# rafaelvp-db/databricks-distributed-deep-learning

Hardware: AMD Instinct MI355X
Metric: ResNet-50 images/sec (whole node) (higher is better)
Workload: dtype bf16

## Files before the change

### csrc/build.py

```python
#!/usr/bin/env python3
from __future__ import annotations

import argparse
import concurrent.futures as cf
import glob
import os
import shutil
import subprocess
import sys

ROOT = os.path.dirname(os.path.dirname(os.path.abspath(__file__)))
CSRC = os.path.join(ROOT, "csrc")
BUILD = os.path.join(ROOT, "build", "native")
OUT_DIR = os.path.join(ROOT, "databricks_distributed_deep_learning_amd", "_native")
OUT = os.path.join(OUT_DIR, "libddl_kernels.so")
HIPCC = os.environ.get("HIPCC", "/opt/rocm/bin/hipcc")
ARCH = os.environ.get("DDL_OFFLOAD_ARCH", "gfx950")

COMMON = ["-O3", "-std=c++17", "-fPIC", f"--offload-arch={ARCH}", "-I", os.path.join(CSRC, "include"),
          "-Wno-unused-result", "-ffp-contract=fast", "-munsafe-fp-atomics"]


def sources():
    return sorted(glob.glob(os.path.join(CSRC, "kernels", "*.hip"))) + \
        sorted(glob.glob(os.path.join(CSRC, "runtime", "*.cpp")))


def headers():
    return glob.glob(os.path.join(CSRC, "include", "*.h")) + glob.glob(os.path.join(CSRC, "kernels", "*.h"))


def obj_for(src):
    return os.path.join(BUILD, os.path.basename(src) + ".o")


def needs(src, obj, hdr_mtime):
    if not os.path.exists(obj):
        return True
    m = os.path.getmtime(obj)
    return os.path.getmtime(src) > m or hdr_mtime > m


_VGPR_FORM = ["-mllvm", "-amdgpu-mfma-vgpr-form"]
EXTRA = {"gemm_big.hip": _VGPR_FORM, "conv3x3.hip": _VGPR_FORM, "skinny_gemm.hip": _VGPR_FORM,
         "stream_gemm.hip": _VGPR_FORM, "gemm_duo.hip": _VGPR_FORM, "conv3_bwd.hip": _VGPR_FORM}


GEMM_SOURCES = ["gemm.hip", "gemm_big.hip", "gemm_duo.hip", "skinny_gemm.hip", "stream_gemm.hip", "conv3x3.hip",
                "conv3_bwd.hip"]


def gemm_src_hash() -> str:
    import hashlib
    h = hashlib.sha256()
    for path in [os.path.join(CSRC, "kernels", n) for n in GEMM_SOURCES] + \
            sorted(glob.glob(os.path.join(CSRC, "include", "*.h"))):
        h.update(os.path.basename(path).encode())
        with open(path, "rb") as f:
            h.update(f.read())
    return h.hexdigest()[:16]


def buildinfo_obj() -> str:
    digest = gemm_src_hash()
    src = os.path.join(BUILD, "buildinfo.cpp")
    obj = src + ".o"
    text = ('extern "C" __attribute__((visibility("default"))) const char* ddl_gemm_src_hash() '
            f'{{ return "{digest}"; }}\n')
    old = open(src).read() if os.path.exists(src) else ""
    if old != text or not os.path.exists(obj):
        with open(src, "w") as f:
            f.write(text)
        r = subprocess.run(["g++", "-O2", "-fPIC", "-c", src, "-o", obj], capture_output=True, text=True)
        if r.returncode != 0:
            raise RuntimeError(f"buildinfo compile failed: {r.stderr}")
    return obj


# ... 63 lines not shown
```

### databricks_distributed_deep_learning_amd/models/layers.py

```python
from __future__ import annotations

import math
from typing import Optional

import torch
import torch.nn as nn

from .. import ops
from ..ops.bridge import BNStats


class Conv2d(nn.Module):

    def __init__(self, cin: int, cout: int, k: int, stride: int = 1, padding: int = 0):
        super().__init__()
        self.cin, self.cout, self.k, self.stride, self.padding = cin, cout, k, stride, padding
        self.weight = nn.Parameter(torch.empty(cout, k, k, cin))
        std = math.sqrt(2.0 / (cout * k * k))
        nn.init.normal_(self.weight, 0.0, std)

    def forward(self, x, grad_residual=None, bn_stats=None, grad_to=None):
        return ops.conv2d(x, self.weight, self.stride, self.padding, grad_residual=grad_residual, bn_stats=bn_stats,
                          grad_to=grad_to)

    def extra_repr(self):
        return f"{self.cin}, {self.cout}, k={self.k}, stride={self.stride}, padding={self.padding}"


class BatchNorm2d(nn.Module):

    def __init__(self, c: int, eps: float = 1e-5, momentum: float = 0.1, relu: bool = False,
                 zero_init: bool = False):
        super().__init__()
        self.c, self.eps, self.momentum, self.relu = c, eps, momentum, relu
        self.weight = nn.Parameter(torch.zeros(c) if zero_init else torch.ones(c))
        self.bias = nn.Parameter(torch.zeros(c))
        self.register_buffer("running_mean", torch.zeros(c))
        self.register_buffer("running_var", torch.ones(c))
        self.register_buffer("num_batches_tracked", torch.tensor(0, dtype=torch.long))
        self._nbt_pending = 0
        self.sync_group = None

    def _flush_nbt(self):
        if self._nbt_pending:
            self.num_batches_tracked.add_(self._nbt_pending)
            self._nbt_pending = 0

    def _save_to_state_dict(self, destination, prefix, keep_vars):
        self._flush_nbt()
        super()._save_to_state_dict(destination, prefix, keep_vars)

    def _load_from_state_dict(self, state_dict, prefix, *args, **kwargs):
        self._nbt_pending = 0
        super()._load_from_state_dict(state_dict, prefix, *args, **kwargs)

    def forward(self, x, residual: Optional[torch.Tensor] = None, residual_grad_to=None, stats=None):
        if self.training:
            self._nbt_pending += 1
        return ops.batch_norm(x, self.weight, self.bias, self.running_mean, self.running_var,
                              self.training, self.momentum, self.eps, self.relu, residual,
                              residual_grad_to=residual_grad_to, stats=stats, group=self.sync_group)

    def _apply(self, fn, recurse=True):
        rm, rv = self.running_mean, self.running_var
        super()._apply(fn, recurse)
        if self.running_mean.dtype != torch.float32:
            self.running_mean = self.running_mean.float()
            self.running_var = self.running_var.float()
        return self

    def extra_repr(self):
        return f"{self.c}, eps={self.eps}, relu={self.relu}"


class Linear(nn.Module):
    def __init__(self, fin: int, fout: int, bias: bool = True, act: Optional[str] = None,
                 init_std: Optional[float] = None):
        super().__init__()
        self.fin, self.fout, self.act = fin, fout, act
        self.weight = nn.Parameter(torch.empty(fout, fin))
        self.bias = nn.Parameter(torch.zeros(fout)) if bias else None
        if init_std is not None:
            nn.init.normal_(self.weight, 0.0, init_std)
        else:
            nn.init.kaiming_uniform_(self.weight, a=math.sqrt(5))
            if self.bias is not None:
                bound = 1.0 / math.sqrt(fin)
                nn.init.uniform_(self.bias, -bound, bound)

    def forward(self, x, grad_residual=None, fuse_dgelu: bool = False, residual=None, residual_grad_to=None):
        return ops.linear(x, self.weight, self.bias, self.act, grad_residual=grad_residual, fuse_dgelu=fuse_dgelu,
                          residual=residual, residual_grad_to=residual_grad_to)

    def extra_repr(self):
        return f"{self.fin}, {self.fout}, bias={self.bias is not None}, act={self.act}"


def conv_bn(conv: "Conv2d", bn: "BatchNorm2d", x, residual=None, grad_residual=None, residual_grad_to=None,
            grad_to=None):
    st = BNStats() if bn.training else None
    y = conv(x, grad_residual=grad_residual, bn_stats=st, grad_to=grad_to)
    return bn(y, residual=residual, residual_grad_to=residual_grad_to, stats=st)


def conv_stats(conv: "Conv2d", bn: "BatchNorm2d", x, grad_residual=None):
    st = BNStats() if bn.training else None
    return conv(x, grad_residual=grad_residual, bn_stats=st), st


def conv_bn_add_bn(conv: "Conv2d", bn: "BatchNorm2d", x, bn2: "BatchNorm2d", y2, st2=None):
    st = BNStats() if bn.training else None
    y = conv(x, bn_stats=st)
    if bn.training and bn2.training and bn.sync_group is None and bn2.sync_group is None and bn.relu \
            and not bn2.relu:
        out = ops.batch_norm_add_bn(y, bn.weight, bn.bias, bn.running_mean, bn.running_var, bn.momentum, bn.eps,
                                    y2, bn2.weight, bn2.bias, bn2.running_mean, bn2.running_var, bn2.momentum,
                                    bn2.eps, st, st2)
        if out is not None:
            bn._nbt_pending += 1
            bn2._nbt_pending += 1
            return out
    return bn(y, residual=bn2(y2, stats=st2), stats=st)


def conv_bn_maxpool(conv: "Conv2d", bn: "BatchNorm2d", x):
    if bn.training and bn.sync_group is None and bn.relu:
        st = BNStats()
        y = conv(x, bn_stats=st)
        out = ops.bn_relu_maxpool(y, bn.weight, bn.bias, bn.running_mean, bn.running_var, bn.momentum, bn.eps, st)
        if out is not None:
            bn._nbt_pending += 1
            return out
        return ops.max_pool2d(bn(y, stats=st), 3, 2, 1)
    return ops.max_pool2d(conv_bn(conv, bn, x), 3, 2, 1)

# ... 49 lines not shown
```

### databricks_distributed_deep_learning_amd/models/resnet.py

```python
from __future__ import annotations

import os
from typing import List, Optional, Type, Union

import torch
import torch.nn as nn

from .. import ops
from ..ops.bridge import GradBridge
from .layers import BatchNorm2d, Conv2d, Linear, conv_bn, conv_bn_add_bn, conv_bn_maxpool, conv_stats


_BRIDGE = os.environ.get("DDL_GRAD_BRIDGE", "1") != "0"


def _bridge(x: torch.Tensor, training: bool):
    return GradBridge() if (_BRIDGE and training and torch.is_grad_enabled() and x.requires_grad) else None


class BasicBlock(nn.Module):
    expansion = 1

    def __init__(self, cin: int, planes: int, stride: int = 1, downsample: Optional[nn.Module] = None,
                 zero_init_residual: bool = False):
        super().__init__()
        self.conv1 = Conv2d(cin, planes, 3, stride, 1)
        self.bn1 = BatchNorm2d(planes, relu=True)
        self.conv2 = Conv2d(planes, planes, 3, 1, 1)
        self.bn2 = BatchNorm2d(planes, relu=True, zero_init=zero_init_residual)
        self.downsample = downsample

    def forward(self, x):
        if self.downsample is None:
            br = _bridge(x, self.training)
            out = conv_bn(self.conv1, self.bn1, x, grad_residual=br)
            return conv_bn(self.conv2, self.bn2, out, residual=x, residual_grad_to=br)
        br = _bridge(x, self.training)
        y_id, st_id = self.downsample.conv_stats(x, grad_residual=br)
        out = conv_bn(self.conv1, self.bn1, x, grad_to=br)
        return conv_bn_add_bn(self.conv2, self.bn2, out, self.downsample.bn, y_id, st_id)


class Bottleneck(nn.Module):
    expansion = 4

    def __init__(self, cin: int, planes: int, stride: int = 1, downsample: Optional[nn.Module] = None,
                 zero_init_residual: bool = False):
        super().__init__()
        self.conv1 = Conv2d(cin, planes, 1)
        self.bn1 = BatchNorm2d(planes, relu=True)
        self.conv2 = Conv2d(planes, planes, 3, stride, 1)
        self.bn2 = BatchNorm2d(planes, relu=True)
        self.conv3 = Conv2d(planes, planes * 4, 1)
        self.bn3 = BatchNorm2d(planes * 4, relu=True, zero_init=zero_init_residual)
        self.downsample = downsample

    def forward(self, x):
        if self.downsample is None:
            br = _bridge(x, self.training)
            out = conv_bn(self.conv1, self.bn1, x, grad_residual=br)
            out = conv_bn(self.conv2, self.bn2, out)
            return conv_bn(self.conv3, self.bn3, out, residual=x, residual_grad_to=br)
        br = _bridge(x, self.training)
        y_id, st_id = self.downsample.conv_stats(x, grad_residual=br)
        out = conv_bn(self.conv1, self.bn1, x, grad_to=br)
        out = conv_bn(self.conv2, self.bn2, out)
        return conv_bn_add_bn(self.conv3, self.bn3, out, self.downsample.bn, y_id, st_id)


class Downsample(nn.Module):

    def __init__(self, cin: int, cout: int, stride: int):
        super().__init__()
        self.add_module("0", Conv2d(cin, cout, 1, stride, 0))
        self.add_module("1", BatchNorm2d(cout, relu=False))

    @property
    def bn(self):
        return self._modules["1"]

    def conv_stats(self, x, grad_residual=None):
        return conv_stats(self._modules["0"], self._modules["1"], x, grad_residual=grad_residual)

    def forward(self, x, grad_residual=None):
        return conv_bn(self._modules["0"], self._modules["1"], x, grad_residual=grad_residual)


class ResNet(nn.Module):
    def __init__(self, block: Type[Union[BasicBlock, Bottleneck]], layers: List[int], num_classes: int = 1000,
                 zero_init_residual: bool = False, channels_last_input: bool = True):
        super().__init__()
        self.channels_last_input = channels_last_input
        self.inplanes = 64
        self.conv1 = Conv2d(3, 64, 7, 2, 3)
        self.bn1 = BatchNorm2d(64, relu=True)
        self.layer1 = self._make_layer(block, 64, layers[0], 1, zero_init_residual)
        self.layer2 = self._make_layer(block, 128, layers[1], 2, zero_init_residual)
        self.layer3 = self._make_layer(block, 256, layers[2], 2, zero_init_residual)
        self.layer4 = self._make_layer(block, 512, layers[3], 2, zero_init_residual)
        self.fc = Linear(512 * block.expansion, num_classes)

    def _make_layer(self, block, planes, blocks, stride, zir):
        down = None
        if stride != 1 or self.inplanes != planes * block.expansion:
            down = Downsample(self.inplanes, planes * block.expansion, stride)
        mods = [block(self.inplanes, planes, stride, down, zir)]
        self.inplanes = planes * block.expansion
        for _ in range(1, blocks):
            mods.append(block(self.inplanes, planes, 1, None, zir))
        return nn.Sequential(*mods)

    _ddl_direct_reads = ("conv1", "bn1")

    def features(self, x):
        if not self.channels_last_input:
            x = x.permute(0, 2, 3, 1).contiguous()
        x = conv_bn_maxpool(self.conv1, self.bn1, x)
        x = self.layer4(self.layer3(self.layer2(self.layer1(x))))
        return ops.global_avg_pool(x)

    def forward(self, x):
        return self.fc(self.features(x))


def resnet18(num_classes: int = 1000, **kw) -> ResNet:
    return ResNet(BasicBlock, [2, 2, 2, 2], num_classes, **kw)


def resnet34(num_classes: int = 1000, **kw) -> ResNet:
    return ResNet(BasicBlock, [3, 4, 6, 3], num_classes, **kw)


def resnet50(num_classes: int = 1000, **kw) -> ResNet:
    return ResNet(Bottleneck, [3, 4, 6, 3], num_classes, **kw)


def resnet101(num_classes: int = 1000, **kw) -> ResNet:
    return ResNet(Bottleneck, [3, 4, 23, 3], num_classes, **kw)


def resnet152(num_classes: int = 1000, **kw) -> ResNet:
    return ResNet(Bottleneck, [3, 8, 36, 3], num_classes, **kw)
# ... 19 lines not shown
```

### databricks_distributed_deep_learning_amd/ops/_lib.py

```python
from __future__ import annotations

import ctypes
import os
from typing import Optional

import torch

_PKG_DIR = os.path.dirname(os.path.dirname(os.path.abspath(__file__)))
LIB_PATH = os.environ.get("DDL_NATIVE_LIB") or os.path.join(_PKG_DIR, "_native", "libddl_kernels.so")

_lib: Optional[ctypes.CDLL] = None
_load_error: Optional[str] = None
_mode = os.environ.get("DDL_NATIVE", "auto").lower()


class NativeUnavailable(RuntimeError):
    pass


def set_mode(mode: str) -> None:
    global _mode
    if mode not in ("auto", "on", "off"):
        raise ValueError(mode)
    _mode = mode
# ... 90 lines not shown
    "ddl_bn_relu_maxpool": [I, P, P, P, P, P, P, I, I, I, I, I, I, P],
    "ddl_bn_bwd_pool_nblk": [],
    "ddl_bn_bwd_pool": [I, P, P, P, P, P, P, P, I, I, I, I, I, I, P, P, P, P, P, I, P],
    "ddl_bn_bwd_coef_from_partials": [I, P, I, P, L, P, P, L, I, P, P, P, I, P],
    "ddl_bn_bwd_apply_coef": [I, P, P, P, P, P, L, I, P, P],
    "ddl_bn_fwd_from_partials": [I, P, I, L, I, P, P, P, P, F, F, P, P, P, P, P, L],
    "ddl_conv_w_dgrad": [P, P, I, I, I, I, I, I, P, P, P],
    "ddl_conv_w_dgrad_batch": [P, P, I, P],
    "ddl_gelu_bwd_colsum": [I, P, P, P, L, I, P, P, I, I, P],
    "ddl_acc_f32": [I, P, P, L, P],
    "ddl_tanh_bwd": [I, P, P, P, L, P],
    "ddl_copy2d": [I, P, L, L, L, P, L, L, L, P],
    "ddl_add_into": [I, P, P, L, P],
    "ddl_zero": [P, L, P],
    "ddl_rows_add_row": [I, P, P, P, L, L, P],
    "ddl_seq_prepend_add": [I, P, P, P, P, L, L, L, P],
    "ddl_sort_ids_ok": [L, L],
    "ddl_sort_ids": [P, L, P, P, P],
    "ddl_drain_acc": [I, P, P, L, P],
    "ddl_acc_grad": [I, P, P, L, I, I, P],
    "ddl_softmax_topk": [I, P, L, I, I, P, P, P, P],
    "ddl_gemm_conv_multi": [I, I, P, P, P, P, P, L, I, P, P],
    "ddl_conv3x3": [P, P, P, I, I, I, I, I, P, P, P, P, P, P, I, P],
    "ddl_conv3x3_wgrad": [P, P, P, I, I, I, I, I, P, L, I, I, I, P],
    "ddl_stem_wgrad": [P, P, P, I, I, I, I, I, I, I, P, L, I, I, I, P],
    "ddl_stem_fwd": [P, P, P, I, I, I, I, P, I, P],
    "ddl_s2d_input": [P, I, I, I, I, I, P, I, I, P],
    "ddl_s2d_weight": [P, I, I, I, I, P, I, I, P],
    "ddl_skinny_gemm": [P, P, P, L, I, I, P, P, P, P, P, P, I, P],
    "ddl_stream_gemm": [P, P, P, L, I, I, P, P, P, P, P, P, I, P],
    "ddl_stream_wgrad_ws": [I, I],
    "ddl_conv3_bwd_grid": [L, I],
    "ddl_conv3_bwd": [P, P, P, P, P, P, P, P, P, P, P, P, P, P, L, P, I, I, L, I, I, I, P],
    "ddl_bn_bwd": [I, P, P, P, P, P, P, L, I, I, P, P, P, P, P, P, I, P],
    "ddl_ln_supported": [I],
    "ddl_ln_fwd": [I, P, P, L, P, P, P, P, P, L, I, F, U64, F, P],
    "ddl_ln_bwd_nblk": [L],
    "ddl_ln_bwd": [I, P, P, P, L, P, P, P, P, P, P, P, L, I, I, P, U64, F, P, P, P, P],
    "ddl_gelu_fwd": [I, P, P, L, P],
    "ddl_gelu_bwd": [I, P, P, P, L, P],
    "ddl_dropout": [I, P, P, L, U64, F, P],
    "ddl_colsum_nblk": [L],
    "ddl_colsum": [I, P, L, I, P, P, I, I, P],
    "ddl_softmax_ce": [I, P, P, L, I, P, P, P, P],
    "ddl_scale_by": [I, P, P, P, L, P],
    "ddl_maxpool_fwd": [I, P, P, P, I, I, I, I, I, I, I, I, I, P],
    "ddl_maxpool_bwd": [I, P, P, P, I, I, I, I, I, I, I, I, I, P],
    "ddl_avgpool_fwd": [I, P, P, I, I, I, P],
    "ddl_avgpool_bwd": [I, P, P, I, I, I, P],
    "ddl_embedding_fwd": [I, P, P, P, L, I, P],
    "ddl_embedding_bwd": [I, P, P, P, P, L, L, I, I, P],
    "ddl_embedding_bwd_sorted": [I, P, P, P, P, P, L, I, I, P],
    "ddl_sgd_step": [I, P, P, I, P, P, P, I, P, F, F, F, I, I, P],
    "ddl_adamw_step": [I, P, P, I, P, P, P, P, I, P, F, F, F, F, F, F, F, F, F, P],
    "ddl_lamb_step": [I, P, P, I, P, P, P, P, I, P, F, F, F, F, F, F, F, F, F, P, P],
    "ddl_sumsq": [I, P, L, P, P],
    "ddl_lamb_phase1": [I, P, P, P, P, P, I, P, F, F, F, F, F, F, F, F, P, P],
    "ddl_lamb_phase2": [P, I, P, P, P, P, I, F, F, F, F, F, P, P],
}
_fns = {}


def fn(name: str):
    f = _fns.get(name)
    if f is None:
        f = getattr(get(), name)
# ... 85 lines not shown
```

### databricks_distributed_deep_learning_amd/ops/_native_conv.py

```python
from __future__ import annotations

import ctypes
import os

import torch
import torch.nn.functional as F

from . import _lib
from ._lib import grad_ready, grad_sink
from ._native_gemm import MODE_CONV, MODE_CONVW, MODE_NN, MODE_NT, MODE_TN, gemm, plan, stats_rows_max
from ._native_norm import _BN_BWD_EPI, _BN_BWD_EPI_RES


def _desc(N, H, W, C, P, Q, stride, h_off, w_off, h_step, w_step, R, S, OH, OW, ostep=1, oa=0, ob=0):
    return [N, H, W, C, P, Q, stride, h_off, w_off, h_step, w_step, R, S, OH, OW, ostep, oa, ob]


STATS_MIN_K = int(os.environ.get("DDL_BN_STATS_MIN_K", "0"))
_DGRAD_NT = os.environ.get("DDL_DGRAD_NT", "1") != "0"


_CONV3X3 = os.environ.get("DDL_CONV3X3", "1") != "0"


# ... 406 lines not shown
    if sink is not None and (not sink.is_contiguous() or sink.dtype not in (torch.bfloat16, torch.float32)):
        return None
    wt = _w_dgrad(w, [0], [0], param).view(C, K)
    dx = torch.empty(N, H, W_, C, dtype=x.dtype, device=x.device)
    dw = sink if sink is not None else torch.empty(K, 1, 1, C, dtype=x.dtype, device=x.device)
    G = _lib.fn("ddl_conv3_bwd_grid")(M, 0)
    part = torch.empty(max(stats_rows_max(M), 1024) * 2 * C + 64 * C, dtype=torch.float32, device=x.device)
    wpart = torch.empty(G * K * C, dtype=torch.bfloat16, device=x.device)
    rc = _lib.fn("ddl_conv3_bwd")(dz.data_ptr(), x3.data_ptr(), mean3.data_ptr(), istd3.data_ptr(), coef.data_ptr(),
                                  x.data_ptr(), bnb.x.data_ptr(), _lib.p(bnb.mask), bnb.mean.data_ptr(),
                                  bnb.istd.data_ptr(), wt.data_ptr(), dx.data_ptr(), part.data_ptr(),
                                  wpart.data_ptr(), wpart.numel(), dw.data_ptr(), int(dw.dtype == torch.float32),
                                  int(sink is not None), M, K, C, 0, _lib.stream())
    if rc == -1:
        return None
    if rc < 0:
        raise RuntimeError(f"ddl_conv3_bwd failed: {rc}")
    bnb.set(dx, part, rc)
    return dx, (None if sink is not None else dw)


def _conv3_materialise(parked, dy):
    from .bridge import Conv3Fold
    dz, x3, mean3, istd3, coef = parked
    C = x3.shape[-1]
    dx3 = torch.empty_like(x3)
    _lib.call("ddl_bn_bwd_apply_coef", 1, dz.data_ptr(), x3.data_ptr(), mean3.data_ptr(), istd3.data_ptr(),
              coef.data_ptr(), x3.numel() // C, C, dx3.data_ptr())
    if Conv3Fold.is_parked(parked, dy):
        return dx3
    return (dy - dz.view_as(dy)) + dx3.view_as(dy)


class _Conv(torch.autograd.Function):
    @staticmethod
    def forward(ctx, x, w, stride, pad, bridge=None, stats=None, grad_to=None):
        ctx.w_param = w
        ctx.bridge = bridge
        ctx.grad_to = grad_to
        ctx.c3 = None
        ctx.bnb = getattr(x, "_ddl_bnb", None) if grad_to is None else None
        x = x.contiguous()
        w = w.contiguous()
        ctx.stride, ctx.pad = stride, pad
        ctx.save_for_backward(x, w)
        y = _fwd(x, w, stride, pad, stats=stats)
        if _conv3_fold_ok(x, w, stride, pad) and y.is_contiguous():
            from .bridge import Conv3Fold
            ctx.c3 = y._ddl_c3 = Conv3Fold()
        return y

    @staticmethod
    def backward(ctx, dy):
        x, w = ctx.saved_tensors
        dy = dy.contiguous()
        dx = dw = None
        parked = ctx.c3.take() if ctx.c3 is not None else None
        if parked is not None:
            from .bridge import Conv3Fold
            if (Conv3Fold.is_parked(parked, dy) and ctx.needs_input_grad[0] and ctx.needs_input_grad[1]
                    and ctx.bridge is None and ctx.grad_to is None):
                sink = grad_sink(ctx.w_param)
                if sink is not None and sink.shape != w.shape:
                    sink = None
                out = _conv3_bwd_fused(parked, x, w, ctx.bnb, ctx.w_param, sink)
                if out is not None:
                    ctx.bnb = None
                    if sink is not None:
                        grad_ready(ctx.w_param)
                    return out[0], out[1], None, None, None, None, None
            dy = _conv3_materialise(parked, dy)
        del parked
        fork = _lib.fork_event() if ctx.needs_input_grad[1] else None
        if ctx.needs_input_grad[0]:
            res = ctx.bridge.take() if ctx.bridge is not None else None
            if res is not None:
                res = res.contiguous().view(x.shape)
            dx = _dgrad(dy, w, x.shape, ctx.stride, ctx.pad, residual=res, bnb=ctx.bnb, param=ctx.w_param)
            ctx.bnb = None
# ... 216 lines not shown
```

### databricks_distributed_deep_learning_amd/ops/_native_norm.py

```python
from __future__ import annotations

import os
from types import SimpleNamespace
from typing import Optional

import torch

from . import _lib
from ._native_elementwise import new_seed
from ._lib import call, dcode, grad_ready, grad_sink, p

_BN_BWD_EPI = os.environ.get("DDL_BN_BWD_EPI", "1") != "0"
_BN_BWD_EPI_RES = os.environ.get("DDL_BN_BWD_EPI", "1") not in ("0", "nores")


def _bn_supported(C: int) -> bool:
    return C % 8 == 0 and 256 % (C // 8) == 0


def _group_sum(row: torch.Tensor, group) -> None:
    import torch.distributed as dist
    from ..parallel import comm as _comm
    eng = _comm.active()
    if eng is not None and row.is_cuda and (group is None or group is dist.group.WORLD
                                            or dist.get_world_size(group) == eng.world):
        eng.wait_upto(eng.all_reduce(row))
        return
    dist.all_reduce(row, op=dist.ReduceOp.SUM, group=group)


def _bn_train_stats(x, weight, bias, running_mean, running_var, momentum, eps, given, stats) -> None:
    C = x.shape[-1]
    M = x.numel() // C
    dt = dcode(x)
    f32 = dict(dtype=torch.float32, device=x.device)
    if given is not None:
        part, nblk = given
        ws = torch.empty(-(-nblk // 32) * 2 * C, **f32) if nblk > 32 else None
        call("ddl_bn_fwd_from_partials", dt, p(part), nblk, M, C, p(weight), p(bias), p(running_mean),
             p(running_var), float(momentum), float(eps), p(stats[0]), p(stats[1]), p(stats[2]), p(stats[3]),
             p(ws), 0 if ws is None else ws.numel())
    else:
        nblk = _lib.fn("ddl_bn_stats_nblk")(M, C)
        part = torch.empty(nblk * 2 * C, **f32)
        call("ddl_bn_fwd_train", dt, p(x), M, C, p(weight), p(bias), p(running_mean), p(running_var),
             float(momentum), float(eps), p(part), p(stats[0]), p(stats[1]), p(stats[2]), p(stats[3]))


class _BatchNormTrain(torch.autograd.Function):
    @staticmethod
    def forward(ctx, x, weight, bias, running_mean, running_var, momentum, eps, relu, residual, bridge=None,
                pre=None, group=None):
        ctx.bridge = bridge
        ctx.group = group
        ctx.c3 = _conv3_hint(x) if group is None else None
        x = x.contiguous()
        C = x.shape[-1]
        M = x.numel() // C
        dt = dcode(x)
        f32 = dict(dtype=torch.float32, device=x.device)
        stats = torch.empty(4, C, **f32)
        given = pre.take_for(x) if pre is not None else None
        if group is not None:
            import torch.distributed as dist
            world = dist.get_world_size(group)
            if given is not None:
                part, nblk = given
                ws = torch.empty(-(-nblk // 32) * 2 * C, **f32)
            else:
                nblk = _lib.fn("ddl_bn_stats_nblk")(M, C)
                part = torch.empty((nblk + -(-nblk // 32)) * 2 * C, **f32)
                call("ddl_bn_stats_partials", dt, p(x), M, C, p(part))
                ws = None
            row = torch.empty(2 * C, **f32)
            call("ddl_bn_rows_sum", p(part), nblk, 2 * C, p(row), p(ws))
            _group_sum(row, group)
            call("ddl_bn_fwd_from_partials", dt, p(row), 1, M * world, C, p(weight), p(bias), p(running_mean),
                 p(running_var), float(momentum), float(eps), p(stats[0]), p(stats[1]), p(stats[2]), p(stats[3]),
                 None, 0)
            ctx.m_total = M * world
        else:
            _bn_train_stats(x, weight, bias, running_mean, running_var, momentum, eps, given, stats)
        res = residual.contiguous() if residual is not None else None
        y = torch.empty_like(x)
        mask = torch.empty(x.numel() // 8, dtype=torch.uint8, device=x.device) if relu else None
        call("ddl_bn_apply", dt, p(x), p(res), p(stats[2]), p(stats[3]), p(y), x.numel(), C, int(relu), p(mask))
        ctx.relu = bool(relu)
        ctx.has_res = residual is not None
        ctx.params = (weight, bias)
        ctx.save_for_backward(x, mask, weight, stats)
        ctx.bnb = None
        if _BN_BWD_EPI and x.dtype == torch.bfloat16:
            from .bridge import BNBackward
            ctx.bnb = BNBackward(x, mask, stats[0], stats[1])
            y._ddl_bnb = ctx.bnb
        return y

    @staticmethod
    def backward(ctx, dy):
        x, mask, weight, stats = ctx.saved_tensors
        dx, dgamma, dbeta, dres = _bn_backward(ctx, dy, x, mask, weight, stats)
        return dx, dgamma, dbeta, None, None, None, None, None, dres, None, None, None


def _conv3_hint(x):
    hint = getattr(x, "_ddl_c3", None)
    if hint is None or not x.is_contiguous() or x.dtype != torch.bfloat16 or not x.requires_grad:
        return None
    return hint


def _bn_backward(ctx, dy, x, mask, weight, stats):
    dy = dy.contiguous()
    C = x.shape[-1]
    M = x.numel() // C
    nblk = _lib.fn("ddl_bn_bwd_nblk")(M, C)
    f32 = dict(dtype=torch.float32, device=x.device)
    part = torch.empty((nblk + -(-nblk // 32)) * 2 * C, **f32)
    coef = torch.empty(3 * C, **f32)
    sg, sb = grad_sink(ctx.params[0]), grad_sink(ctx.params[1])
    direct = sg is not None and sb is not None
    if direct:
        dgamma, dbeta = sg, sb
    else:
        dgamma = torch.empty_like(weight) if weight is not None else None
        dbeta = torch.empty_like(weight) if weight is not None else None
    given = ctx.bnb.take_for(dy) if ctx.bnb is not None else None
    ctx.bnb = None
    c3 = getattr(ctx, "c3", None)
    fold = c3 is not None and given is not None and ctx.group is None and weight is not None
    dx = None if fold else torch.empty_like(x)
    dres = torch.empty_like(x) if ctx.has_res and (given is None or ctx.group is not None) else None
    if given is not None:
        gpart, nrows = given
        if ctx.group is not None:
# ... 138 lines not shown
_FUSED_STEM_BWD = os.environ.get("DDL_FUSED_STEM_BWD", "0") != "0"


def batch_norm_add_bn(x, weight, bias, running_mean, running_var, momentum, eps, x2, weight2, bias2,
                      running_mean2, running_var2, momentum2, eps2, pre=None, pre2=None):
    C = x.shape[-1]
    if (not _bn_supported(C) or x.dtype not in (torch.bfloat16, torch.float32) or x2.dtype != x.dtype
            or x2.shape != x.shape or weight is None or weight2 is None):
        return None
    if weight.dtype != x.dtype:
        weight, bias = weight.to(x.dtype), bias.to(x.dtype)
    if weight2.dtype != x.dtype:
        weight2, bias2 = weight2.to(x.dtype), bias2.to(x.dtype)
    return _BatchNormAddBNTrain.apply(x, weight, bias, running_mean, running_var, momentum, eps, x2, weight2, bias2,
                                      running_mean2, running_var2, momentum2, eps2, pre, pre2)


class _BatchNormEval(torch.autograd.Function):

    @staticmethod
    def forward(ctx, x, weight, bias, running_mean, running_var, eps, relu, residual):
        x = x.contiguous()
        C = x.shape[-1]
        coeff = torch.empty(2, C, dtype=torch.float32, device=x.device)
        call("ddl_bn_eval_coeffs", dcode(x), C, p(weight), p(bias), p(running_mean), p(running_var), float(eps),
             p(coeff[0]), p(coeff[1]))
        y = torch.empty_like(x)
        res = residual.contiguous() if residual is not None else None
        call("ddl_bn_apply", dcode(x), p(x), p(res), p(coeff[0]), p(coeff[1]), p(y), x.numel(), C, int(relu), None)
        return y


def batch_norm(x, weight, bias, running_mean, running_var, training, momentum, eps, relu, residual, bridge=None,
               pre=None, group=None):
    from .norm import batch_norm_reference, sync_batch_norm_reference
    C = x.shape[-1]
    if not _bn_supported(C) or x.dtype not in (torch.bfloat16, torch.float32):
        if training and group is not None:
            return sync_batch_norm_reference(x, weight, bias, running_mean, running_var, momentum, eps, relu,
                                             residual, group)
        return batch_norm_reference(x, weight, bias, running_mean, running_var, training, momentum, eps, relu,
                                    residual)
    if weight is not None and weight.dtype != x.dtype:
        weight, bias = weight.to(x.dtype), bias.to(x.dtype)
    if training:
        return _BatchNormTrain.apply(x, weight, bias, running_mean, running_var, momentum, eps, relu, residual,
                                     bridge, pre, group)
    if torch.is_grad_enabled() and (x.requires_grad or (weight is not None and weight.requires_grad)):
        return batch_norm_reference(x, weight, bias, running_mean, running_var, False, momentum, eps, relu,
                                    residual)
    return _BatchNormEval.apply(x, weight, bias, running_mean, running_var, eps, relu, residual)


class _LayerNorm(torch.autograd.Function):
    @staticmethod
    def forward(ctx, x, weight, bias, eps, residual, drop_p, bridge=None, grad_from=None):
        ctx.bias_param = getattr(x, "_ddl_bias_param", None)
        ctx.grad_from = grad_from
        x = x.contiguous()
        H = x.shape[-1]
        rows = x.numel() // H
        res = residual.contiguous() if residual is not None else None
        res_rows = res.numel() // H if res is not None else rows
        stats = torch.empty(2, rows, dtype=torch.float32, device=x.device)
        y = torch.empty_like(x)
        seed = new_seed() if drop_p > 0.0 else 0
        call("ddl_ln_fwd", dcode(x), p(x), p(res), res_rows, p(weight), p(bias), p(y), p(stats[0]), p(stats[1]),
             rows, H, float(eps), seed, float(drop_p))
        ctx.seed, ctx.drop_p = seed, float(drop_p)
        ctx.bridge = bridge
        ctx.res_shape = residual.shape if residual is not None else None
        ctx.params = (weight, bias)
        ctx.res_rows = res_rows
        ctx.save_for_backward(x, res, weight, stats)
        return y

    @staticmethod
    def backward(ctx, dy):
        x, res, weight, stats = ctx.saved_tensors
        dy = dy.contiguous()
# ... 81 lines not shown
```

### databricks_distributed_deep_learning_amd/ops/bridge.py

```python
from __future__ import annotations

import os
from typing import Optional

import torch

CONV3_FUSED = os.environ.get("DDL_CONV3_BWD_FUSED", "1") != "0"
CONV3_SHAPES = ((256, 64),)


class GradBridge:
    __slots__ = ("grad", "closed")

    def __init__(self):
        self.grad: Optional[torch.Tensor] = None
        self.closed = False

    def put(self, g: torch.Tensor) -> None:
        if self.grad is not None:
            raise RuntimeError("GradBridge: gradient already pending (bridge reused within one backward?)")
        self.grad = g

    def offer(self, g: torch.Tensor) -> bool:
        if self.closed:
            return False
        self.put(g)
        return True

    def take(self) -> Optional[torch.Tensor]:
        g, self.grad = self.grad, None
        self.closed = True
        return g


class _BridgeJoin(torch.autograd.Function):

    @staticmethod
    def forward(ctx, x, bridge):
        ctx.bridge = bridge
        return x.view_as(x)

# ... 37 lines not shown
        self.nrows = 0

    def set(self, dz: torch.Tensor, part: torch.Tensor, nrows: int) -> None:
        self.dz, self.part, self.nrows = dz, part, nrows

    def take_for(self, g: torch.Tensor):
        dz, part, nrows = self.dz, self.part, self.nrows
        self.dz = self.part = None
        if dz is None or dz.data_ptr() != g.data_ptr() or dz.numel() != g.numel():
            return None
        return part, nrows


class Conv3Fold:
    __slots__ = ("parked",)

    def __init__(self):
        self.parked = None

    def park(self, dz: torch.Tensor, x: torch.Tensor, mean: torch.Tensor, istd: torch.Tensor,
             coef: torch.Tensor) -> None:
        if self.parked is not None:
            raise RuntimeError("Conv3Fold: a gradient is already parked (hint reused within one backward?)")
        self.parked = (dz, x, mean, istd, coef)

    def take(self):
        parked, self.parked = self.parked, None
        return parked

    @staticmethod
    def is_parked(parked, g: torch.Tensor) -> bool:
        dz = parked[0]
        return dz.data_ptr() == g.data_ptr() and dz.numel() == g.numel() and dz.dtype == g.dtype
```

### databricks_distributed_deep_learning_amd/ops/norm.py

```python
from __future__ import annotations

from typing import Optional

import torch
import torch.nn.functional as F

from . import _lib


def batch_norm_reference(x, weight, bias, running_mean, running_var, training: bool,
                         momentum: float = 0.1, eps: float = 1e-5, relu: bool = False,
                         residual: Optional[torch.Tensor] = None):
    C = x.shape[-1]
    xf = x.reshape(-1, C)
    if training:
        y = F.batch_norm(xf.float(), running_mean, running_var, weight.float() if weight is not None else None,
                         bias.float() if bias is not None else None, True, momentum, eps)
    else:
        y = F.batch_norm(xf.float(), running_mean, running_var, weight.float() if weight is not None else None,
                         bias.float() if bias is not None else None, False, momentum, eps)
    y = y.view_as(x)
    if residual is not None:
        y = y + residual.float()
    if relu:
        y = torch.relu(y)
    return y.to(x.dtype)


def sync_batch_norm_reference(x, weight, bias, running_mean, running_var, momentum: float = 0.1,
                              eps: float = 1e-5, relu: bool = False, residual: Optional[torch.Tensor] = None,
                              group=None):
    import torch.distributed as dist
    from torch.distributed.nn.functional import all_reduce
    C = x.shape[-1]
    xf = x.reshape(-1, C).float()
    world = dist.get_world_size(group)
    n = xf.shape[0] * world
    st = all_reduce(torch.cat([xf.sum(0), (xf * xf).sum(0)]), op=dist.ReduceOp.SUM, group=group)
    mean = st[:C] / n
    var = (st[C:] / n - mean * mean).clamp_min(0)
    y = (xf - mean) * torch.rsqrt(var + eps)
    if weight is not None:
        y = y * weight.float() + bias.float()
    with torch.no_grad():
        running_mean.mul_(1 - momentum).add_(mean.detach(), alpha=momentum)
        running_var.mul_(1 - momentum).add_(var.detach() * (n / max(1, n - 1)), alpha=momentum)
    y = y.view_as(x)
    if residual is not None:
        y = y + residual.float()
    if relu:
        y = torch.relu(y)
    return y.to(x.dtype)


def batch_norm(x, weight, bias, running_mean, running_var, training: bool, momentum: float = 0.1,
               eps: float = 1e-5, relu: bool = False, residual: Optional[torch.Tensor] = None,
               residual_grad_to=None, stats=None, group=None):
    if _lib.use_native(x):
        from . import _native_norm
        return _native_norm.batch_norm(x, weight, bias, running_mean, running_var, training,
                                       momentum, eps, relu, residual, residual_grad_to, stats, group)
    if training and group is not None:
        return sync_batch_norm_reference(x, weight, bias, running_mean, running_var, momentum, eps, relu,
                                         residual, group)
    return batch_norm_reference(x, weight, bias, running_mean, running_var, training, momentum, eps,
                                relu, residual)


def layer_norm_reference(x, weight, bias, eps: float = 1e-12, residual: Optional[torch.Tensor] = None):
    h = x if residual is None else x + residual
    y = F.layer_norm(h.float(), (h.shape[-1],), weight.float() if weight is not None else None,
                     bias.float() if bias is not None else None, eps)
    return y.to(x.dtype)


def layer_norm(x, weight, bias, eps: float = 1e-12, residual: Optional[torch.Tensor] = None,
               dropout: float = 0.0, residual_grad_to=None, grad_from=None):
    if _lib.use_native(x):
        from . import _native_norm
        return _native_norm.layer_norm(x, weight, bias, eps, residual, dropout, residual_grad_to, grad_from)
    if dropout > 0.0:
        x = F.dropout(x, dropout, True)
    from .bridge import join
    return layer_norm_reference(join(x, grad_from), weight, bias, eps, residual)


def batch_norm_add_bn(x, weight, bias, running_mean, running_var, momentum, eps, x2, weight2, bias2,
                      running_mean2, running_var2, momentum2, eps2, stats=None, stats2=None):
    if not _lib.use_native(x, x2):
        return None
    from . import _native_norm
    return _native_norm.batch_norm_add_bn(x, weight, bias, running_mean, running_var, momentum, eps, x2, weight2,
                                          bias2, running_mean2, running_var2, momentum2, eps2, stats, stats2)

# ... 7 lines not shown
```

Baseline: 12940.

## Fuse BN-apply+residual+ReLU with next block's 1x1 conv1 forward

Adds a HIP kernel that applies batch-norm scale/shift, residual add and ReLU for the 256-channel bottleneck output. It writes the activation and ReLU mask, then immediately runs the following block's 256->64 1x1 conv on the tile still in LDS with MFMA, emitting the conv output and per-block column stats. The next Conv2d claims the precomputed result through a hint attached to the tensor. This is meant to avoid re-reading the activation from HBM and to save a separate GEMM launch. The cost is extra bookkeeping that ties validity to weight version and pointer identity. It only applies when the model runs without sync BN, so it is skipped when a sync group is set, and it is also skipped during graph capture.

```diff
diff --git a/csrc/build.py b/csrc/build.py
--- a/csrc/build.py
+++ b/csrc/build.py
@@ -43,7 +43,8 @@
 
 _VGPR_FORM = ["-mllvm", "-amdgpu-mfma-vgpr-form"]
 EXTRA = {"gemm_big.hip": _VGPR_FORM, "conv3x3.hip": _VGPR_FORM, "skinny_gemm.hip": _VGPR_FORM,
-         "stream_gemm.hip": _VGPR_FORM, "gemm_duo.hip": _VGPR_FORM, "conv3_bwd.hip": _VGPR_FORM}
+         "stream_gemm.hip": _VGPR_FORM, "gemm_duo.hip": _VGPR_FORM, "conv3_bwd.hip": _VGPR_FORM,
+         "apply_conv1.hip": _VGPR_FORM}
 
 
 GEMM_SOURCES = ["gemm.hip", "gemm_big.hip", "gemm_duo.hip", "skinny_gemm.hip", "stream_gemm.hip", "conv3x3.hip",
diff --git a/csrc/kernels/apply_conv1.hip b/csrc/kernels/apply_conv1.hip
--- /dev/null
+++ b/csrc/kernels/apply_conv1.hip
@@ -0,0 +1,265 @@
+#include "ddl_lds.h"
+
+#include <algorithm>
+
+namespace {
+
+constexpr int NW = 8, NTH = NW * 64;
+constexpr int TM = 32;
+constexpr int DPT = 4, SPT = 4;
+
+struct AcParams {
+    const bf16_t* z3;
+    const bf16_t* res;
+    const float* scale;
+    const float* shift;
+    const bf16_t* w;
+    bf16_t* out;
+    uint8_t* mask;
+    bf16_t* z1;
+    float* colstats;
+    long M;
+    int tiles, chunk;
+    uint32_t out_bytes, mask_bytes, z1_bytes;
+};
+
+__device__ __forceinline__ void wait_vm4(int n) {
+    switch (n) {
+        case 4: asm volatile("s_waitcnt vmcnt(4)" ::: "memory"); break;
+        case 8: asm volatile("s_waitcnt vmcnt(8)" ::: "memory"); break;
+        case 12: asm volatile("s_waitcnt vmcnt(12)" ::: "memory"); break;
+        default: asm volatile("s_waitcnt vmcnt(0)" ::: "memory"); break;
+    }
+}
+
+__device__ __forceinline__ void ds_write1(uint32_t addr, uint32_t v) {
+    asm volatile("ds_write_b8 %0, %1" ::"v"(addr), "v"(v) : "memory");
+}
+
+__device__ __forceinline__ u32x4 apply8(bf16x8 zv, bf16x8 rv, const float* sc, const float* sh, uint32_t& bits) {
+    const u32x4 zw = __builtin_bit_cast(u32x4, zv), rw = __builtin_bit_cast(u32x4, rv);
+    u32x4 o;
+    bits = 0;
+#pragma unroll
+    for (int i = 0; i < 4; ++i) {
+        const float t0 = fmaxf(__builtin_fmaf(lo_f(zw[i]), sc[2 * i], sh[2 * i]) + lo_f(rw[i]), 0.f);
+        const float t1 = fmaxf(__builtin_fmaf(hi_f(zw[i]), sc[2 * i + 1], sh[2 * i + 1]) + hi_f(rw[i]), 0.f);
+        o[i] = pack2bf(t0, t1);
+        bits |= (lo_f(o[i]) > 0.f ? 1u : 0u) << (2 * i);
+        bits |= (hi_f(o[i]) > 0.f ? 1u : 0u) << (2 * i + 1);
+    }
+    return o;
+}
+
+template <int C, int N, int NBUF>
+__global__ __launch_bounds__(NTH, 1) void apply_conv1_k(AcParams p) {
+    static_assert(C == 256 && N == 64 && NBUF == 3, "shape");
+    constexpr int WBYTES = N * C * 2, ZBYTES = TM * C * 2, YBYTES = TM * N * 2, MBYTES = TM * C / 8;
+    constexpr int O_Z = 0, O_R = ZBYTES, O_Y = 2 * ZBYTES, O_MK = O_Y + YBYTES;
+    constexpr int BUFB = O_MK + MBYTES;
+    constexpr int LDS = WBYTES + NBUF * BUFB;
+    static_assert(LDS <= 160 * 1024, "LDS");
+    __shared__ __attribute__((aligned(16))) char smem[LDS];
+    const int tid = threadIdx.x, lane = tid & 63, wv = __builtin_amdgcn_readfirstlane(tid >> 6);
+    const int g = lane >> 4, r16 = lane & 15;
+    const uint32_t lds0 = (uint32_t)(uintptr_t)smem;
+    const __amdgpu_buffer_rsrc_t ors = rsrc(p.out, p.out_bytes), mrs = rsrc(p.mask, p.mask_bytes),
+                                 yrs = rsrc(p.z1, p.z1_bytes);
+    const int t0 = blockIdx.x * p.chunk, t1 = min(p.tiles, t0 + p.chunk);
+
+    const int tc = tid & 31, tr = tid >> 5;
+    float sc[8], sh[8];
+    load8(p.scale + tc * 8, sc);
+    load8(p.shift + tc * 8, sh);
+
+    auto prefetch = [&](int t, int buf) {
+        char* base = smem + WBYTES + buf * BUFB;
+        const long m0 = (long)t * TM;
+#pragma unroll
+        for (int qq = 0; qq < 2; ++qq) {
+            const int q = qq * NW + wv, r = q * 2 + (lane >> 5), c = (lane & 31) ^ (r & 15);
+            const long gr = min(m0 + r, p.M - 1);
+            glds16_nt(p.z3 + gr * C + c * 8, base + O_Z + q * 1024);
+            glds16_nt(p.res + gr * C + c * 8, base + O_R + q * 1024);
+        }
+    };
+#pragma unroll
+    for (int qq = 0; qq < N / 2 / NW; ++qq) {
+        const int q = qq * NW + wv, r = q * 2 + (lane >> 5), c = (lane & 31) ^ (r & 15);
+        glds16_nt(p.w + (long)r * C + c * 8, smem + q * 1024);
+    }
+#pragma unroll
+    for (int u = 0; u < NBUF - 1; ++u)
+        if (t0 + u < t1) prefetch(t0 + u, u);
+
+    const uint32_t toff = tr * (C * 2) + ((tc ^ tr) << 4);
+    const uint32_t tmk = tr * (C / 8) + tc;
+
+    const int dj = wv & 3;
+    const bool gw = wv < 4;
+    uint32_t aoff[2][C / 32], boff[C / 32];
+#pragma unroll
+    for (int kk = 0; kk < C / 32; ++kk) {
+        const int rb = 16 * dj + r16;
+        boff[kk] = lds0 + rb * (C * 2) + (((kk * 4 + g) ^ (rb & 15)) << 4);
+#pragma unroll
+        for (int i = 0; i < 2; ++i) {
+            const int ra = 16 * i + r16;
+            aoff[i][kk] = ra * (C * 2) + (((kk * 4 + g) ^ (ra & 15)) << 4);
+        }
+    }
+    uint32_t coff[2];
+#pragma unroll
+    for (int i = 0; i < 2; ++i) {
+        const int drow = 16 * i + r16;
+        coff[i] = drow * (N * 2) + (((2 * dj + (g >> 1)) ^ (drow & 7)) << 4) + (g & 1) * 8;
+    }
+    float st_s[4] = {0.f, 0.f, 0.f, 0.f}, st_q[4] = {0.f, 0.f, 0.f, 0.f};
+
+    int buf = 0;
+    for (int t = t0; t < t1; ++t) {
+        wait_vm4(min(NBUF - 1, t - t0) * SPT + min(NBUF - 2, t1 - 1 - t) * DPT);
+        __builtin_amdgcn_s_barrier();
+        if (t + NBUF - 1 < t1) prefetch(t + NBUF - 1, buf == 0 ? NBUF - 1 : buf - 1);
+        const uint32_t img = lds0 + WBYTES + buf * BUFB;
+        const long m0 = (long)t * TM;
+
+        {
+            const bf16x8 z0 = ds_read16(img + O_Z + toff), z1 = ds_read16(img + O_Z + toff + 16 * C * 2);
+            const bf16x8 x0 = ds_read16(img + O_R + toff), x1 = ds_read16(img + O_R + toff + 16 * C * 2);
+            LGKM0();
+            __builtin_amdgcn_sched_barrier(0);
+            uint32_t b0, b1;
+            ds_write16(img + O_Z + toff, apply8(z0, x0, sc, sh, b0));
+            ds_write16(img + O_Z + toff + 16 * C * 2, apply8(z1, x1, sc, sh, b1));
+            ds_write1(img + O_MK + tmk, b0);
+            ds_write1(img + O_MK + tmk + 16 * (C / 8), b1);
+            LGKM0();
+            __builtin_amdgcn_s_barrier();
+        }
+
+        {
+            u32x4 d[2];
+            int row[2];
+#pragma unroll
+            for (int qq = 0; qq < 2; ++qq) {
+                const int q = qq * NW + wv;
+                row[qq] = q * 2 + (lane >> 5);
+                d[qq] = __builtin_bit_cast(u32x4, ds_read16(img + O_Z + row[qq] * (C * 2) +
+                                                           (((lane & 31) ^ (row[qq] & 15)) << 4)));
+            }
+            const uint32_t mb = wv * 128 + (lane & 31) * 4;
+            const uint32_t mw = ds_read32(img + O_MK + mb);
+            LGKM0();
+            __builtin_amdgcn_sched_barrier(0);
+#pragma unroll
+            for (int qq = 0; qq < 2; ++qq) {
+                const long grow = m0 + row[qq];
+                const uint32_t off = grow < p.M ? (uint32_t)((grow * C + (lane & 31) * 8) * 2) : 0x80000000u;
+                __builtin_amdgcn_raw_buffer_store_b128(d[qq], ors, (int)off, 0, 0);
+            }
+            const long mrow = m0 + (mb >> 5);
+            const uint32_t moff = (lane < 32 && mrow < p.M) ? (uint32_t)(m0 * (C / 8) + mb) : 0x80000000u;
+            __builtin_amdgcn_raw_buffer_store_b32(mw, mrs, (int)moff, 0, 0);
+        }
+
+        if (gw) {
+            f32x4 acc[2] = {{0.f, 0.f, 0.f, 0.f}, {0.f, 0.f, 0.f, 0.f}};
+#pragma unroll
+            for (int k2 = 0; k2 < C / 32; k2 += 4) {
+                bf16x8 af[2][4], bfr[4];
+#pragma unroll
+                for (int u = 0; u < 4; ++u) {
+                    af[0][u] = ds_read16(img + O_Z + aoff[0][k2 + u]);
+                    af[1][u] = ds_read16(img + O_Z + aoff[1][k2 + u]);
+                    bfr[u] = ds_read16(boff[k2 + u]);
+                }
+                LGKM0();
+                __builtin_amdgcn_sched_barrier(0);
+#pragma unroll
+                for (int u = 0; u < 4; ++u) {
+                    acc[0] = __builtin_amdgcn_mfma_f32_16x16x32_bf16(bfr[u], af[0][u], acc[0], 0, 0, 0);
+                    acc[1] = __builtin_amdgcn_mfma_f32_16x16x32_bf16(bfr[u], af[1][u], acc[1], 0, 0, 0);
+                }
+                __builtin_amdgcn_sched_barrier(0);
+            }
+#pragma unroll
+            for (int i = 0; i < 2; ++i) {
+                const uint32_t lo = pack2bf(acc[i][0], acc[i][1]), hi = pack2bf(acc[i][2], acc[i][3]);
+                ds_write8(img + O_Y + coff[i], make_uint2(lo, hi));
+                if (m0 + 16 * i + r16 < p.M) {
+                    const float tq[4] = {lo_f(lo), hi_f(lo), lo_f(hi), hi_f(hi)};
+#pragma unroll
+                    for (int e = 0; e < 4; ++e) {
+                        st_s[e] += tq[e];
+                        st_q[e] += tq[e] * tq[e];
+                    }
+                }
+            }
+        }
+        LGKM0();
+        __builtin_amdgcn_s_barrier();
+        {
+            const int row = 4 * wv + (lane >> 4), pc = lane & 15;
+            const uint2 d = ds_read8(img + O_Y + row * (N * 2) + (((pc >> 1) ^ (row & 7)) << 4) + (pc & 1) * 8);
+            LGKM0();
+            __builtin_amdgcn_sched_barrier(0);
+            const long grow = m0 + row;
+            const uint32_t off = grow < p.M ? (uint32_t)((grow * N + pc * 4) * 2) : 0x80000000u;
+            __builtin_amdgcn_raw_buffer_store_b64(__builtin_bit_cast(u32x2, d), yrs, (int)off, 0, 0);
+        }
+        buf = buf + 1 == NBUF ? 0 : buf + 1;
+    }
+
+    if (gw) {
+#pragma unroll
+        for (int e = 0; e < 4; ++e) {
+            const float a = row16_sum(st_s[e]), b = row16_sum(st_q[e]);
+            if (r16 == 0) {
+                const int col = 16 * dj + 4 * g + e;
+                p.colstats[(long)blockIdx.x * 2 * N + col] = a;
+                p.colstats[(long)blockIdx.x * 2 * N + N + col] = b;
+            }
+        }
+    }
+}
+
+}
+
+DDL_API int ddl_apply_conv1_grid(long M, int grid) {
+    const int tiles64 = (int)((M + 63) / 64);
+    const int g = std::min(grid > 0 ? std::min(grid, 256) : 256, tiles64);
+    const int chunk64 = (tiles64 + g - 1) / g;
+    return (tiles64 + chunk64 - 1) / chunk64;
+}
+
+DDL_API int ddl_apply_conv1(const void* z3, const void* res, const float* scale, const float* shift, const void* w,
+                            void* out, void* mask, void* z1, float* colstats, long M, int C, int N, int grid,
+                            hipStream_t st) {
+    if (C != 256 || N != 64 || M < 1 || M * (long)C * 2 >= (1l << 31)) return -1;
+    if (!z3 || !res || !scale || !shift || !w || !out || !mask || !z1 || !colstats) return -1;
+    for (const void* q : {z3, res, w, (const void*)out, (const void*)z1, (const void*)scale, (const void*)shift})
+        if ((uintptr_t)q & 15) return -1;
+    if ((uintptr_t)mask & 3) return -1;
+    AcParams p{};
+    p.z3 = (const bf16_t*)z3;
+    p.res = (const bf16_t*)res;
+    p.scale = scale;
+    p.shift = shift;
+    p.w = (const bf16_t*)w;
+    p.out = (bf16_t*)out;
+    p.mask = (uint8_t*)mask;
+    p.z1 = (bf16_t*)z1;
+    p.colstats = colstats;
+    p.M = M;
+    p.tiles = (int)((M + TM - 1) / TM);
+    const int G = ddl_apply_conv1_grid(M, grid);
+    p.chunk = 2 * (((int)((M + 63) / 64) + G - 1) / G);
+    p.out_bytes = (uint32_t)(M * C * 2);
+    p.mask_bytes = (uint32_t)(M * (C / 8));
+    p.z1_bytes = (uint32_t)(M * N * 2);
+    hipLaunchKernelGGL((apply_conv1_k<256, 64, 3>), dim3(G), dim3(NTH), 0, st, p);
+    const hipError_t e = hipGetLastError();
+    if (e != hipSuccess) return -2 - (int)e;
+    return G;
+}
diff --git a/databricks_distributed_deep_learning_amd/models/layers.py b/databricks_distributed_deep_learning_amd/models/layers.py
--- a/databricks_distributed_deep_learning_amd/models/layers.py
+++ b/databricks_distributed_deep_learning_amd/models/layers.py
@@ -54,12 +54,14 @@
         self._nbt_pending = 0
         super()._load_from_state_dict(state_dict, prefix, *args, **kwargs)
 
-    def forward(self, x, residual: Optional[torch.Tensor] = None, residual_grad_to=None, stats=None):
+    def forward(self, x, residual: Optional[torch.Tensor] = None, residual_grad_to=None, stats=None,
+                next_conv: Optional["Conv2d"] = None):
         if self.training:
             self._nbt_pending += 1
         return ops.batch_norm(x, self.weight, self.bias, self.running_mean, self.running_var,
                               self.training, self.momentum, self.eps, self.relu, residual,
-                              residual_grad_to=residual_grad_to, stats=stats, group=self.sync_group)
+                              residual_grad_to=residual_grad_to, stats=stats, group=self.sync_group,
+                              next_conv_weight=next_conv.weight if next_conv is not None and self.training else None)
 
     def _apply(self, fn, recurse=True):
         rm, rv = self.running_mean, self.running_var
@@ -97,10 +99,10 @@
 
 
 def conv_bn(conv: "Conv2d", bn: "BatchNorm2d", x, residual=None, grad_residual=None, residual_grad_to=None,
-            grad_to=None):
+            grad_to=None, next_conv: Optional["Conv2d"] = None):
     st = BNStats() if bn.training else None
     y = conv(x, grad_residual=grad_residual, bn_stats=st, grad_to=grad_to)
-    return bn(y, residual=residual, residual_grad_to=residual_grad_to, stats=st)
+    return bn(y, residual=residual, residual_grad_to=residual_grad_to, stats=st, next_conv=next_conv)
 
 
 def conv_stats(conv: "Conv2d", bn: "BatchNorm2d", x, grad_residual=None):
diff --git a/databricks_distributed_deep_learning_amd/models/resnet.py b/databricks_distributed_deep_learning_amd/models/resnet.py
--- a/databricks_distributed_deep_learning_amd/models/resnet.py
+++ b/databricks_distributed_deep_learning_amd/models/resnet.py
@@ -54,18 +54,33 @@
         self.conv3 = Conv2d(planes, planes * 4, 1)
         self.bn3 = BatchNorm2d(planes * 4, relu=True, zero_init=zero_init_residual)
         self.downsample = downsample
+        self._fold_next = ()
 
     def forward(self, x):
         if self.downsample is None:
             br = _bridge(x, self.training)
             out = conv_bn(self.conv1, self.bn1, x, grad_residual=br)
             out = conv_bn(self.conv2, self.bn2, out)
-            return conv_bn(self.conv3, self.bn3, out, residual=x, residual_grad_to=br)
+            nxt = self._fold_next[0].conv1 if self._fold_next else None
+            return conv_bn(self.conv3, self.bn3, out, residual=x, residual_grad_to=br, next_conv=nxt)
         br = _bridge(x, self.training)
         y_id, st_id = self.downsample.conv_stats(x, grad_residual=br)
         out = conv_bn(self.conv1, self.bn1, x, grad_to=br)
         out = conv_bn(self.conv2, self.bn2, out)
         return conv_bn_add_bn(self.conv3, self.bn3, out, self.downsample.bn, y_id, st_id)
+
+
+def link_conv1_fold(blocks) -> list:
+    from ..ops.bridge import APPLY_CONV1_SHAPES
+    pairs = []
+    for i in range(len(blocks) - 1):
+        a, b = blocks[i], blocks[i + 1]
+        ok = (isinstance(a, Bottleneck) and isinstance(b, Bottleneck) and a.downsample is None
+              and b.downsample is None and (b.conv1.cout, b.conv1.cin) in APPLY_CONV1_SHAPES)
+        a._fold_next = (b,) if ok else ()
+        if ok:
+            pairs.append((i, i + 1))
+    return pairs
 
 
 class Downsample(nn.Module):
@@ -108,6 +123,7 @@
         self.inplanes = planes * block.expansion
         for _ in range(1, blocks):
             mods.append(block(self.inplanes, planes, 1, None, zir))
+        link_conv1_fold(mods)
         return nn.Sequential(*mods)
 
     _ddl_direct_reads = ("conv1", "bn1")
diff --git a/databricks_distributed_deep_learning_amd/ops/_lib.py b/databricks_distributed_deep_learning_amd/ops/_lib.py
--- a/databricks_distributed_deep_learning_amd/ops/_lib.py
+++ b/databricks_distributed_deep_learning_amd/ops/_lib.py
@@ -146,6 +146,8 @@
     "ddl_stream_wgrad_ws": [I, I],
     "ddl_conv3_bwd_grid": [L, I],
     "ddl_conv3_bwd": [P, P, P, P, P, P, P, P, P, P, P, P, P, P, L, P, I, I, L, I, I, I, P],
+    "ddl_apply_conv1_grid": [L, I],
+    "ddl_apply_conv1": [P, P, P, P, P, P, P, P, P, L, I, I, I, P],
     "ddl_bn_bwd": [I, P, P, P, P, P, P, L, I, I, P, P, P, P, P, P, I, P],
     "ddl_ln_supported": [I],
     "ddl_ln_fwd": [I, P, P, L, P, P, P, P, P, L, I, F, U64, F, P],
diff --git a/databricks_distributed_deep_learning_amd/ops/_native_conv.py b/databricks_distributed_deep_learning_amd/ops/_native_conv.py
--- a/databricks_distributed_deep_learning_amd/ops/_native_conv.py
+++ b/databricks_distributed_deep_learning_amd/ops/_native_conv.py
@@ -462,6 +462,19 @@
     return (dy - dz.view_as(dy)) + dx3.view_as(dy)
 
 
+def _conv1_folded(hint, x, w, stride, pad, stats):
+    given = hint.claim(x, w)
+    K, R, S, C = w.shape
+    if given is None or R != 1 or S != 1 or stride != 1 or pad != 0:
+        return None
+    z1, part, nblk = given
+    if tuple(z1.shape) != (*x.shape[:3], K) or z1.dtype != x.dtype:
+        return None
+    if stats is not None:
+        stats.set(z1, part, nblk)
+    return z1
+
+
 class _Conv(torch.autograd.Function):
     @staticmethod
     def forward(ctx, x, w, stride, pad, bridge=None, stats=None, grad_to=None):
@@ -470,11 +483,14 @@
         ctx.grad_to = grad_to
         ctx.c3 = None
         ctx.bnb = getattr(x, "_ddl_bnb", None) if grad_to is None else None
+        c1 = getattr(x, "_ddl_c1", None)
         x = x.contiguous()
         w = w.contiguous()
         ctx.stride, ctx.pad = stride, pad
         ctx.save_for_backward(x, w)
-        y = _fwd(x, w, stride, pad, stats=stats)
+        y = _conv1_folded(c1, x, w, stride, pad, stats) if c1 is not None else None
+        if y is None:
+            y = _fwd(x, w, stride, pad, stats=stats)
         if _conv3_fold_ok(x, w, stride, pad) and y.is_contiguous():
             from .bridge import Conv3Fold
             ctx.c3 = y._ddl_c3 = Conv3Fold()
diff --git a/databricks_distributed_deep_learning_amd/ops/_native_norm.py b/databricks_distributed_deep_learning_amd/ops/_native_norm.py
--- a/databricks_distributed_deep_learning_amd/ops/_native_norm.py
+++ b/databricks_distributed_deep_learning_amd/ops/_native_norm.py
@@ -47,10 +47,43 @@
              float(momentum), float(eps), p(part), p(stats[0]), p(stats[1]), p(stats[2]), p(stats[3]))
 
 
+def _apply_conv1_ok(x, res, relu, group, fold_w) -> bool:
+    from . import bridge as B
+    if fold_w is None or not B.APPLY_CONV1_FUSED or group is not None or not relu or res is None:
+        return False
+    C = x.shape[-1]
+    if fold_w.dim() != 4 or (fold_w.shape[0], fold_w.shape[3]) not in B.APPLY_CONV1_SHAPES \
+            or fold_w.shape[1] != 1 or fold_w.shape[2] != 1 or fold_w.shape[3] != C:
+        return False
+    return (x.is_cuda and x.dtype == torch.bfloat16 and x.dim() == 4 and res.dtype == torch.bfloat16
+            and res.shape == x.shape and res.is_contiguous() and fold_w.is_cuda and fold_w.dtype == torch.bfloat16
+            and fold_w.is_contiguous() and x.numel() * 2 < 2 ** 31 and x.data_ptr() % 16 == 0
+            and res.data_ptr() % 16 == 0 and fold_w.data_ptr() % 16 == 0
+            and not torch.cuda.is_current_stream_capturing())
+
+
+def _apply_conv1(x, res, scale, shift, y, mask, w):
+    from .bridge import Conv1Fold
+    N_, H, W_, C = x.shape
+    K = w.shape[0]
+    M = N_ * H * W_
+    G = _lib.fn("ddl_apply_conv1_grid")(M, 0)
+    z1 = torch.empty(N_, H, W_, K, dtype=x.dtype, device=x.device)
+    part = torch.empty(G * 2 * K, dtype=torch.float32, device=x.device)
+    rc = _lib.fn("ddl_apply_conv1")(x.data_ptr(), res.data_ptr(), scale.data_ptr(), shift.data_ptr(), w.data_ptr(),
+                                    y.data_ptr(), mask.data_ptr(), z1.data_ptr(), part.data_ptr(), M, C, K, 0,
+                                    _lib.stream())
+    if rc == -1:
+        return None
+    if rc < 0:
+        raise RuntimeError(f"ddl_apply_conv1 failed: {rc}")
+    return Conv1Fold(y, z1, part, rc, w)
+
+
 class _BatchNormTrain(torch.autograd.Function):
     @staticmethod
     def forward(ctx, x, weight, bias, running_mean, running_var, momentum, eps, relu, residual, bridge=None,
-                pre=None, group=None):
+                pre=None, group=None, fold_w=None):
         ctx.bridge = bridge
         ctx.group = group
         ctx.c3 = _conv3_hint(x) if group is None else None
@@ -84,7 +117,12 @@
         res = residual.contiguous() if residual is not None else None
         y = torch.empty_like(x)
         mask = torch.empty(x.numel() // 8, dtype=torch.uint8, device=x.device) if relu else None
-        call("ddl_bn_apply", dt, p(x), p(res), p(stats[2]), p(stats[3]), p(y), x.numel(), C, int(relu), p(mask))
+        c1 = _apply_conv1(x, res, stats[2], stats[3], y, mask, fold_w) \
+            if _apply_conv1_ok(x, res, relu, group, fold_w) else None
+        if c1 is not None:
+            y._ddl_c1 = c1
+        else:
+            call("ddl_bn_apply", dt, p(x), p(res), p(stats[2]), p(stats[3]), p(y), x.numel(), C, int(relu), p(mask))
         ctx.relu = bool(relu)
         ctx.has_res = residual is not None
         ctx.params = (weight, bias)
@@ -100,7 +138,7 @@
     def backward(ctx, dy):
         x, mask, weight, stats = ctx.saved_tensors
         dx, dgamma, dbeta, dres = _bn_backward(ctx, dy, x, mask, weight, stats)
-        return dx, dgamma, dbeta, None, None, None, None, None, dres, None, None, None
+        return dx, dgamma, dbeta, None, None, None, None, None, dres, None, None, None, None
 
 
 def _conv3_hint(x):
@@ -305,7 +343,7 @@
 
 
 def batch_norm(x, weight, bias, running_mean, running_var, training, momentum, eps, relu, residual, bridge=None,
-               pre=None, group=None):
+               pre=None, group=None, fold_w=None):
     from .norm import batch_norm_reference, sync_batch_norm_reference
     C = x.shape[-1]
     if not _bn_supported(C) or x.dtype not in (torch.bfloat16, torch.float32):
@@ -318,7 +356,7 @@
         weight, bias = weight.to(x.dtype), bias.to(x.dtype)
     if training:
         return _BatchNormTrain.apply(x, weight, bias, running_mean, running_var, momentum, eps, relu, residual,
-                                     bridge, pre, group)
+                                     bridge, pre, group, fold_w)
     if torch.is_grad_enabled() and (x.requires_grad or (weight is not None and weight.requires_grad)):
         return batch_norm_reference(x, weight, bias, running_mean, running_var, False, momentum, eps, relu,
                                     residual)
diff --git a/databricks_distributed_deep_learning_amd/ops/bridge.py b/databricks_distributed_deep_learning_amd/ops/bridge.py
--- a/databricks_distributed_deep_learning_amd/ops/bridge.py
+++ b/databricks_distributed_deep_learning_amd/ops/bridge.py
@@ -7,6 +7,9 @@
 
 CONV3_FUSED = os.environ.get("DDL_CONV3_BWD_FUSED", "1") != "0"
 CONV3_SHAPES = ((256, 64),)
+
+APPLY_CONV1_FUSED = os.environ.get("DDL_APPLY_CONV1_FUSED", "1") != "0"
+APPLY_CONV1_SHAPES = ((64, 256),)
 
 
 class GradBridge:
@@ -110,3 +113,19 @@
     def is_parked(parked, g: torch.Tensor) -> bool:
         dz = parked[0]
         return dz.data_ptr() == g.data_ptr() and dz.numel() == g.numel() and dz.dtype == g.dtype
+
+
+class Conv1Fold:
+    __slots__ = ("z1", "part", "nblk", "w", "version", "ptr", "numel")
+
+    def __init__(self, out: torch.Tensor, z1: torch.Tensor, part: torch.Tensor, nblk: int, w: torch.Tensor):
+        self.z1, self.part, self.nblk = z1, part, nblk
+        self.w, self.version = w, w._version
+        self.ptr, self.numel = out.data_ptr(), out.numel()
+
+    def claim(self, x: torch.Tensor, w: torch.Tensor):
+        z1, part, nblk = self.z1, self.part, self.nblk
+        ok = (z1 is not None and w is self.w and w._version == self.version and x.data_ptr() == self.ptr
+              and x.numel() == self.numel)
+        self.z1 = self.part = self.w = None
+        return (z1, part, nblk) if ok else None
diff --git a/databricks_distributed_deep_learning_amd/ops/norm.py b/databricks_distributed_deep_learning_amd/ops/norm.py
--- a/databricks_distributed_deep_learning_amd/ops/norm.py
+++ b/databricks_distributed_deep_learning_amd/ops/norm.py
@@ -55,11 +55,12 @@
 
 def batch_norm(x, weight, bias, running_mean, running_var, training: bool, momentum: float = 0.1,
                eps: float = 1e-5, relu: bool = False, residual: Optional[torch.Tensor] = None,
-               residual_grad_to=None, stats=None, group=None):
+               residual_grad_to=None, stats=None, group=None, next_conv_weight=None):
     if _lib.use_native(x):
         from . import _native_norm
         return _native_norm.batch_norm(x, weight, bias, running_mean, running_var, training,
-                                       momentum, eps, relu, residual, residual_grad_to, stats, group)
+                                       momentum, eps, relu, residual, residual_grad_to, stats, group,
+                                       next_conv_weight)
     if training and group is not None:
         return sync_batch_norm_reference(x, weight, bias, running_mean, running_var, momentum, eps, relu,
                                          residual, group)
```

Result: no change. 12990 (median of 6 runs) (+0.4%).
